# lh3/miniasm

Hardware: AMD Instinct MI355X
Metric: PAF overlaps processed/sec (hit-filter->trans-reduce->GFA) (higher is better)
Workload: dtype u32

## Files before the change

### include/mahip.h

```cpp
#ifndef MAHIP_H
#define MAHIP_H

#include <stddef.h>
#include <stdint.h>
#include "miniasm_amd.h"

#ifdef __cplusplus
extern "C" {
#endif

typedef struct mahip_ctx mahip_ctx_t;

int mahip_device_count(void);
mahip_ctx_t *mahip_create(int device, void *stream);
void mahip_destroy(mahip_ctx_t *c);
const char *mahip_strerror(void);
int mahip_sync(mahip_ctx_t *c);
int mahip_first_launch(mahip_ctx_t *c);

int mahip_hits_upload(mahip_ctx_t *c, const ma_hit_t *h, size_t n, uint32_t n_seq);
int mahip_hits_adopt(mahip_ctx_t *c, const void *d_hits, size_t n, uint32_t n_seq);
int mahip_set_shard(mahip_ctx_t *c, uint32_t q_beg, uint32_t q_end);
int mahip_hits_balance(mahip_ctx_t *c, int world, uint32_t *bounds);
int mahip_set_shard_bounds(mahip_ctx_t *c, const uint32_t *bounds, int world);
// ... 210 lines not shown
int mahip_useq_plan_last(mahip_ctx_t *c, mahip_useq_plan_info_t *info);
const char *mahip_useq_plan_reason_name(int reason);
int mahip_useq_plan_mem(mahip_ctx_t *c, uint32_t n_utg, const uint32_t *u_n, const uint32_t *u_len, const uint64_t *members, uint32_t n_seq, const char *blob, const uint64_t *off,
                        const void *sub, mahip_useq_plan_info_t *info);
int mahip_useq_plan_download(mahip_ctx_t *c, uint64_t *uoff, mahip_useq_place_t *pl, mahip_useq_want_t *want, char *names);
int mahip_useq_begin_planned(mahip_ctx_t *c);
int mahip_useq_place_text_planned(mahip_ctx_t *c, uint64_t *n_matched, uint64_t *n_dup, uint64_t *n_short, double *laps_ms);
int mahip_useq_stream_begin_planned(mahip_ctx_t *c);
enum { MAHIP_BGZF_OK = 0, MAHIP_BGZF_NOT_BGZF, MAHIP_BGZF_NO_BC, MAHIP_BGZF_PAST_END, MAHIP_BGZF_TRAILING, MAHIP_BGZF_BAD_FLG, MAHIP_BGZF_ISIZE,
       MAHIP_BGZF_BAD_BTYPE, MAHIP_BGZF_STORED_LEN, MAHIP_BGZF_BAD_LENGTHS, MAHIP_BGZF_BAD_SYMBOL, MAHIP_BGZF_DIST_TOO_FAR, MAHIP_BGZF_OUT_OVERFLOW, MAHIP_BGZF_IN_EXHAUSTED,
       MAHIP_BGZF_OUT_SHORT, MAHIP_BGZF_CRC, MAHIP_BGZF_NOMEM, MAHIP_BGZF_NOT_SEEKABLE, MAHIP_BGZF_FORCED, MAHIP_BGZF_EMPTY };
enum { MAHIP_BGZF_HOST = 1, MAHIP_BGZF_DEVICE = 2 };
enum { MAHIP_BGZF_PAF = 1, MAHIP_BGZF_FASTX = 2 };
typedef struct {
	uint64_t n_members, n_empty;
	uint64_t n_stored, n_fixed, n_dynamic;
	uint64_t comp_bytes, text_bytes;
	int reader, reason;
	int64_t first_bad_member;
	double laps_ms[4];
} mahip_bgzf_info_t;
typedef struct { uint64_t in_off, out_off; uint32_t in_len, isize, crc, pad; } mahip_bgzf_member_t;
int mahip_bgzf_load_fd(mahip_ctx_t *c, int fd, size_t nbytes, int target, mahip_bgzf_info_t *info);
int mahip_bgzf_load_mem(mahip_ctx_t *c, const void *comp, size_t nbytes, int target, mahip_bgzf_info_t *info);
int mahip_bgzf_inflate_mem(mahip_ctx_t *c, const void *comp, size_t ncomp, void *out, size_t out_cap, mahip_bgzf_info_t *info);
#define MAHIP_BGZF_RANGE_AHEAD 1
typedef struct {
	uint64_t text_bytes;
	uint64_t beg, end;
	uint64_t first_member, n_members_inflated;
	uint64_t comp_bytes_uploaded;
	int n_rounds;
} mahip_bgzf_range_t;
int mahip_bgzf_load_fd_range(mahip_ctx_t *c, int fd, size_t nbytes, int rank, int world, mahip_bgzf_range_t *range, mahip_bgzf_info_t *info);
int mahip_bgzf_range_mem(mahip_ctx_t *c, const void *comp, size_t ncomp, int rank, int world, void *out, size_t out_cap, mahip_bgzf_range_t *range, mahip_bgzf_info_t *info);
int mahip_text_first_nl(mahip_ctx_t *c, const void *d_text, uint64_t from, uint64_t to, uint64_t *pos);
int mahip_bgzf_last(mahip_ctx_t *c, mahip_bgzf_info_t *out);
void mahip_bgzf_note(mahip_ctx_t *c, const mahip_bgzf_info_t *in);
const char *mahip_bgzf_reason_name(int reason);
enum { MAHIP_GZIP_OK = 0, MAHIP_GZIP_BAD_HEADER, MAHIP_GZIP_MULTI_MEMBER, MAHIP_GZIP_NO_SYNC, MAHIP_GZIP_SYNC_MISMATCH, MAHIP_GZIP_ISIZE,
       MAHIP_GZIP_BAD_BTYPE, MAHIP_GZIP_STORED_LEN, MAHIP_GZIP_BAD_LENGTHS, MAHIP_GZIP_BAD_SYMBOL, MAHIP_GZIP_DIST_TOO_FAR, MAHIP_GZIP_OUT_OVERFLOW, MAHIP_GZIP_IN_EXHAUSTED,
       MAHIP_GZIP_OUT_SHORT, MAHIP_GZIP_CRC, MAHIP_GZIP_NOMEM, MAHIP_GZIP_NOT_SEEKABLE, MAHIP_GZIP_FORCED, MAHIP_GZIP_EMPTY };
#define MAHIP_GZIP_CHUNK_DEFAULT ((size_t)1 << 20)
typedef struct {
	uint64_t comp_bytes, text_bytes;
	uint64_t chunk, n_chunks, n_synced, n_items;
	uint64_t n_stored, n_fixed, n_dynamic;
	int reader, reason;
	int64_t first_bad_item;
	double laps_ms[6];
} mahip_gzip_info_t;
#define MAHIP_GZIP_SAW_FINAL 1u
#define MAHIP_GZIP_ON_CHAIN 2u
typedef struct {
	int64_t sync_bit;
	uint64_t end_bit, out_len;
	uint32_t status, flags;
} mahip_gzip_item_t;
int mahip_gzip_load_fd(mahip_ctx_t *c, int fd, size_t nbytes, int target, size_t chunk, mahip_gzip_info_t *info);
int mahip_gzip_load_mem(mahip_ctx_t *c, const void *comp, size_t nbytes, int target, size_t chunk, mahip_gzip_info_t *info);
int mahip_gzip_inflate_mem(mahip_ctx_t *c, const void *comp, size_t ncomp, size_t chunk, void *out, size_t out_cap, mahip_gzip_info_t *info);
int mahip_gzip_last(mahip_ctx_t *c, mahip_gzip_info_t *out);
void mahip_gzip_note(mahip_ctx_t *c, const mahip_gzip_info_t *in);
const char *mahip_gzip_reason_name(int reason);
uint64_t mahip_gzip_items_download(mahip_ctx_t *c, mahip_gzip_item_t *out, uint64_t cap);
uint32_t mahip_asg_n_arc(mahip_ctx_t *c);
enum { MAHIP_SCAN_ONE_TILE = 0, MAHIP_SCAN_CHAINED = 1, MAHIP_SCAN_THREE_PHASE = 2 };
void mahip_scan_forms(mahip_ctx_t *c, uint64_t out[3]);
int mahip_scan_u32(mahip_ctx_t *c, const uint32_t *d_in, uint32_t *d_out, size_t n, uint32_t *d_total);
uint64_t mahip_asg_trans_inner(mahip_ctx_t *c);
int mahip_asg_download(mahip_ctx_t *c, asg_t *g);

#define MAHIP_BUF_SUB0  0
#define MAHIP_BUF_SUB1  1
#define MAHIP_BUF_RCONT 2
#define MAHIP_BUF_RUSED 3
#define MAHIP_BUF_SDEL  4
int mahip_copy_out(mahip_ctx_t *c, int which, void *d_dst, size_t first, size_t count);
int mahip_copy_in(mahip_ctx_t *c, int which, const void *d_src, size_t first, size_t count);
int mahip_hits_contained_flags(mahip_ctx_t *c, const ma_opt_t *opt);
int mahip_hits_contained_finish(mahip_ctx_t *c, const uint8_t *seq_del, uint32_t *n_seq_new, size_t *n_live);
int mahip_sg_flags(mahip_ctx_t *c, const ma_opt_t *opt, int use_sub, const uint32_t *seq_len, const uint8_t *seq_del);
int mahip_sg_finish(mahip_ctx_t *c, uint32_t *n_arc);
int mahip_asg_export_rows(mahip_ctx_t *c, void *d_dst);
int mahip_asg_import_rows(mahip_ctx_t *c, const void *d_src, const uint32_t *counts, int n_ranks, size_t stride);
int mahip_set_full_input(mahip_ctx_t *c, int full);
int mahip_sg_push_conflicts(mahip_ctx_t *c, uint64_t *n_conf);
int mahip_sg_push_fix(mahip_ctx_t *c);
int mahip_asg_export_rows_push(mahip_ctx_t *c, void *d_dst);
int mahip_asg_import_push_rows(mahip_ctx_t *c, const void *d_src, const uint32_t *counts, int n_ranks, size_t stride);
int mahip_asg_del_trans_range(mahip_ctx_t *c, int fuzz, uint32_t v_beg, uint32_t v_end, uint32_t *n_reduced);
int mahip_asg_flags_out(mahip_ctx_t *c, void *d_dst, size_t first, size_t count);
int mahip_asg_flags_in(mahip_ctx_t *c, const void *d_src, size_t first, size_t count);
int mahip_asg_cleanup(mahip_ctx_t *c, uint32_t *n_arc);

int mahip_comm_unique_id(void *id128);
int mahip_comm_init(mahip_ctx_t *c, const void *id128, int rank, int world);
int mahip_comm_init_shm(mahip_ctx_t *c, const char *name, int rank, int world);
void mahip_comm_destroy(mahip_ctx_t *c);
int mahip_comm_rank(mahip_ctx_t *c);
int mahip_comm_world(mahip_ctx_t *c);
int mahip_comm_active(mahip_ctx_t *c);
int mahip_comm_all_gather(mahip_ctx_t *c, const void *d_send, void *d_recv, size_t bytes_per_rank);
int mahip_comm_all_reduce_max_u8(mahip_ctx_t *c, void *d_buf, size_t n);
int mahip_comm_all_reduce_sum_u64(mahip_ctx_t *c, uint64_t *h_vals, size_t n);
typedef struct {
	void *user;
	int (*all_gather)(void *user, const void *send, void *recv, size_t bytes);
	int (*all_reduce_max_u8)(void *user, void *buf, size_t n);
	int (*all_reduce_sum_u64)(void *user, uint64_t *vals, size_t n);
	int (*all_reduce_sum_u32)(void *user, void *buf, size_t n);
	int (*all_to_all_v)(void *user, const void *send, void *recv, const uint64_t *bytes);
} mahip_comm_ext_t;
int mahip_comm_init_ext(mahip_ctx_t *c, int rank, int world, const mahip_comm_ext_t *ext);
int mahip_comm_all_reduce_sum_u32(mahip_ctx_t *c, void *d_buf, size_t n);
int mahip_comm_all_to_all_v(mahip_ctx_t *c, const void *d_send, void *d_recv, const uint64_t *bytes);
int mahip_comm_all_gather_u64(mahip_ctx_t *c, const uint64_t *h_vals, size_t n, uint64_t *h_out);
int mahip_comm_barrier(mahip_ctx_t *c);
int mahip_xbuf(mahip_ctx_t *c, int slot, size_t bytes, void **d_ptr);

#define MAHIP_TEXT_PAF 1
#define MAHIP_TEXT_SG  2
#define MAHIP_TEXT_BED 3
#define MAHIP_TEXT_UG  4
#define MAHIP_TEXT_ROAD_HOST   1
#define MAHIP_TEXT_ROAD_DEVICE 2
#define MAHIP_TEXT_OK        0
#define MAHIP_TEXT_SWITCHED_OFF 1
#define MAHIP_TEXT_NOMEM     2
#define MAHIP_TEXT_NO_NAMES  3
#define MAHIP_TEXT_NO_UG     4
#define MAHIP_TEXT_NO_SEQ    5
#define MAHIP_TEXT_SEQ_NUL   6
#define MAHIP_TEXT_TOO_MANY  7
typedef struct {
	int kind, road, reason;
	uint64_t n_records;
	uint64_t n_lines;
	uint64_t text_bytes;
	uint64_t n_slabs, slab_records;
	uint64_t max_name;
	uint64_t n_slow_lines;
	double laps_ms[4];
	uint64_t n_seq_bytes;
	uint64_t seq_chunk;
} mahip_text_info_t;
typedef int (*mahip_text_sink_t)(void *arg, const char *text, size_t n);
int mahip_text_names(mahip_ctx_t *c, const char *blob, const uint64_t *off, uint32_t n_seq, const uint8_t *del);
int mahip_text_prepare(mahip_ctx_t *c, int kind, int have_sub, mahip_text_info_t *info);
int mahip_text_emit(mahip_ctx_t *c, mahip_text_sink_t sink, void *arg, mahip_text_info_t *info);
int mahip_text_dump(mahip_ctx_t *c, int kind, int have_sub, mahip_text_sink_t sink, void *arg, mahip_text_info_t *info);
int mahip_text_last(mahip_ctx_t *c, mahip_text_info_t *info);
int mahip_text_prepare_ug(mahip_ctx_t *c, int have_sub, const asg_arc_t *links, uint32_t n_links, int with_seq, mahip_text_info_t *info);
int mahip_text_format_mem(mahip_ctx_t *c, int kind, const void *records, uint64_t n_records, const void *sub, uint32_t n_seq, const uint8_t *del,
                          const char *blob, const uint64_t *off, uint64_t slab, char **text, size_t *len, mahip_text_info_t *info);
int mahip_text_format_ug_mem(mahip_ctx_t *c, uint32_t n_utg, const uint32_t *u_n, const uint32_t *u_len, const uint32_t *u_start, const uint32_t *u_end, const uint64_t *members,
                             const asg_arc_t *links, uint32_t n_links, const uint32_t *counts, const void *sub, uint32_t n_seq, int with_seq, const char *arena, uint64_t arena_bytes,
                             const char *blob, const uint64_t *off, uint64_t slab, char **text, size_t *len, mahip_text_info_t *info);
int mahip_text_enabled(void);

int mahip_prof_enable(mahip_ctx_t *c, int enable);
int mahip_prof_reset(mahip_ctx_t *c);
typedef struct { const char *name; uint64_t launches; double total_ms; double alg_bytes; } mahip_prof_t;
int mahip_prof_get(mahip_ctx_t *c, mahip_prof_t *out, int max);
int mahip_mark(mahip_ctx_t *c, int slot);
int mahip_marks_ms(mahip_ctx_t *c, int first, int n, float *ms);
// ... 17 lines not shown
```

### miniasm_amd/csrc/graph.hip

```cpp
#include "mahip_internal.hpp"
#include <type_traits>

#define DEAD 0x80000000u
#define ADEL 0x80000000u

struct HitColsG { const uint32_t *qid, *qs, *qe, *tn, *ts, *te, *ml, *bl; };
struct ArcCols { uint32_t *u, *v, *len, *ol; };

static HitColsG gcols_of(mahip_ctx *c)
{
	HitColsG h;
	h.qid = P<uint32_t>(c->col[0]); h.qs = P<uint32_t>(c->col[1]); h.qe = P<uint32_t>(c->col[2]); h.tn = P<uint32_t>(c->col[3]);
	h.ts = P<uint32_t>(c->col[4]); h.te = P<uint32_t>(c->col[5]); h.ml = P<uint32_t>(c->col[6]); h.bl = P<uint32_t>(c->col[7]);
	return h;
}
static ArcCols arcs_of(mahip_ctx *c, int g)
{
	ArcCols a;
	a.u = P<uint32_t>(c->au[g]); a.v = P<uint32_t>(c->av[g]); a.len = P<uint32_t>(c->alen[g]); a.ol = P<uint32_t>(c->aol[g]);
	return a;
}
static int reserve_arcs(mahip_ctx *c, size_t n)
{
	for (int g = 0; g < 2; ++g) {
		CHK(dev_reserve(c, c->au[g], (n + 4) * 4)); CHK(dev_reserve(c, c->av[g], (n + 4) * 4));
		CHK(dev_reserve(c, c->alen[g], (n + 4) * 4)); CHK(dev_reserve(c, c->aol[g], (n + 4) * 4));
	}
	CHK(dev_reserve(c, c->keep, (n + 16) * 4)); CHK(dev_reserve(c, c->pos, (n + 16) * 4));
	return 0;
}

__global__ __launch_bounds__(256) void k_sg_seq(const uint2 *__restrict__ sub, const uint8_t *__restrict__ r_del, const uint32_t *__restrict__ seq_len,
                                                 const uint8_t *__restrict__ seq_del, uint32_t n_seq, uint32_t *__restrict__ slen, uint8_t *__restrict__ sdel)
{
	uint32_t r = blockIdx.x * 256 + threadIdx.x;
	if (r >= n_seq) return;
	uint32_t len; int del;
	if (sub) { uint2 s = sub[r]; len = s.y - (s.x & 0x7fffffffu); del = s.x >> 31; }
	else len = seq_len[r], del = 0;
	if (seq_del) del |= seq_del[r];
	if (r_del) del |= r_del[r];
	slen[r] = len; sdel[r] = (uint8_t)del;
}

#define SG_TILE 16384u

__device__ __forceinline__ int sg_candidate(const HitColsG &h, size_t i, const uint32_t *__restrict__ slen, int max_hang, float int_frac, int min_ovlp,
                                            const uint8_t *__restrict__ lazy_del, mc_arc_t *x, uint32_t *q_, uint32_t *t_, int *self_rc)
{
	const uint32_t q = h.qid[i];
	if (lazy_del && lazy_del[q]) return -100;
	if (h.bl[i] & DEAD) return -100;
	const uint32_t t = h.tn[i];
	if (lazy_del && lazy_del[t]) return -100;
	uint32_t qs = h.qs[i], qe = h.qe[i], ts = h.ts[i], te = h.te[i];
	int rev = h.ml[i] >> 31;
	*q_ = q; *t_ = t;
	*self_rc = q == t && qs == ts && qe == te && rev;
	return mc_hit2arc(q, qs, qe, t, ts, te, rev, (int)slen[q], (int)slen[t], max_hang, int_frac, min_ovlp, x);
}

__global__ __launch_bounds__(256) void k_sg_arcs(HitColsG h, size_t n, const uint32_t *__restrict__ slen, uint8_t *__restrict__ sdel,
                                                  int max_hang, float int_frac, int min_ovlp, unsigned long long *__restrict__ ctr, const uint8_t *__restrict__ lazy_del,
                                                  unsigned long long *__restrict__ cmask)
{
	uint32_t mx = 0, n_live = 0;
	for (size_t base = (size_t)blockIdx.x * 256; base < n; base += (size_t)gridDim.x * 256) {
		const size_t i = base + threadIdx.x;
		int cand = 0;
		if (i < n) {
			mc_arc_t x;
			uint32_t q = 0, t = 0;
			int self_rc = 0, r = sg_candidate(h, i, slen, max_hang, int_frac, min_ovlp, lazy_del, &x, &q, &t, &self_rc);
			if (r != -100) {
				++n_live;
				if (r >= 0) {
					if (q == t) { if (self_rc) sdel[q] = 1; }
					else cand = 1, mx = x.len > mx ? x.len : mx;
				} else if (r == MC_HT_QCONT) sdel[q] = 1;
			}
		}
		const unsigned long long m = wv_ballot(cand);
		if ((threadIdx.x & 63) == 0) cmask[i >> 6] = m;
	}
	blk_max_u64(&ctr[CT_MAXLEN], mx);
	blk_add_u64(&ctr[CT_LIVE], n_live);
}

#ifndef SG_DENSE
#define SG_DENSE 6
#endif
__device__ __forceinline__ unsigned long long wv_bcast_u64(unsigned long long x, int src) { return (unsigned long long)__shfl((uint32_t)(x >> 32), src, 64) << 32 | __shfl((uint32_t)x, src, 64); }

__global__ __launch_bounds__(256) void k_sg_emit(HitColsG h, size_t n, const uint32_t *__restrict__ slen, const uint8_t *__restrict__ sdel,
                                                  int max_hang, float int_frac, int min_ovlp, const unsigned long long *cmask,
                                                  uint32_t *__restrict__ tile_cnt, const uint32_t *__restrict__ tile_off, ArcCols out, uint32_t *__restrict__ aslot,
                                                  uint32_t *__restrict__ wpos, unsigned long long *kmask)
{
	__shared__ uint32_t s_w[4];
	const unsigned lane = threadIdx.x & 63;
	const size_t w = (size_t)blockIdx.x * 256 + threadIdx.x, n_words = (n + 63) >> 6, w0 = w - lane;
	unsigned long long m = w < n_words ? cmask[w] : 0ull, kept = 0;
	uint32_t cnt = 0;
	const bool dense = __popcll(m) >= SG_DENSE;
	const unsigned long long dense_lanes = wv_ballot(dense);
	for (unsigned long long dl = dense_lanes; dl; dl &= dl - 1) {
		const int l = __ffsll((long long)dl) - 1;
		const unsigned long long ml = wv_bcast_u64(m, l);
		const size_t i = ((w0 + (size_t)l) << 6) + lane;
		const int k = (ml >> lane & 1ull) && i < n && !sdel[h.qid[i]] && !sdel[h.tn[i]];
		const unsigned long long kb = wv_ballot(k);
		if ((int)lane == l) kept = kb, cnt = (uint32_t)__popcll(kb);
	}
	if (!dense)
		for (unsigned long long rest = m; rest; rest &= rest - 1) {
			const int b = __ffsll((long long)rest) - 1;
			const size_t i = (w << 6) + (size_t)b;
			if (i < n && !sdel[h.qid[i]] && !sdel[h.tn[i]]) kept |= 1ull << b, ++cnt;
		}
	uint32_t tot, ex = block_excl_scan_256(cnt, s_w, &tot);
	if (!out.u) { if (threadIdx.x == 0) tile_cnt[blockIdx.x] = tot; return; }
	uint32_t p = tile_off[blockIdx.x] + ex;
	if (wpos && w < n_words) { wpos[w] = p; kmask[w] = kept; }
	for (unsigned long long dl = dense_lanes; dl; dl &= dl - 1) {
		const int l = __ffsll((long long)dl) - 1;
		const unsigned long long kl = wv_bcast_u64(kept, l);
		const uint32_t pl = __shfl(p, l, 64);
		if (kl >> lane & 1ull) {
			const size_t i = ((w0 + (size_t)l) << 6) + lane;
			const uint32_t pp = pl + (uint32_t)__popcll(kl & wv_lt(lane));
			mc_arc_t x;
			uint32_t q = 0, t = 0;
			int self_rc = 0;
			sg_candidate(h, i, slen, max_hang, int_frac, min_ovlp, nullptr, &x, &q, &t, &self_rc);
			out.u[pp] = x.u; out.v[pp] = x.v; out.len[pp] = x.len; out.ol[pp] = x.ol;
			if (aslot) aslot[pp] = (uint32_t)i;
		}
	}
	if (!dense)
		for (; kept; kept &= kept - 1, ++p) {
			const size_t i = (w << 6) + (size_t)(__ffsll((long long)kept) - 1);
			mc_arc_t x;
			uint32_t q = 0, t = 0;
			int self_rc = 0;
			sg_candidate(h, i, slen, max_hang, int_frac, min_ovlp, nullptr, &x, &q, &t, &self_rc);
			out.u[p] = x.u; out.v[p] = x.v; out.len[p] = x.len; out.ol[p] = x.ol;
			if (aslot) aslot[p] = (uint32_t)i;
		}
}

__global__ __launch_bounds__(256) void k_arc_keep(ArcCols a, size_t n, const uint8_t *__restrict__ sdel, uint32_t *__restrict__ keep, int use_keep_in)
{
	size_t i = (size_t)blockIdx.x * 256 + threadIdx.x;
	if (i >= n) return;
	int k = use_keep_in ? (int)keep[i] : 1;
	if (k) k = !(a.ol[i] & ADEL) && !sdel[a.u[i] >> 1] && !sdel[a.v[i] >> 1];
	keep[i] = k;
}

__global__ __launch_bounds__(256) void k_arc_compact(ArcCols in, size_t n, const uint32_t *__restrict__ keep, const uint32_t *__restrict__ pos, ArcCols out)
{
	size_t i = (size_t)blockIdx.x * 256 + threadIdx.x;
	if (i < n && keep[i]) {
		uint32_t p = pos[i];
		out.u[p] = in.u[i]; out.v[p] = in.v[i]; out.len[p] = in.len[i]; out.ol[p] = in.ol[i];
	}
}
// ... 697 lines not shown
}
__global__ __launch_bounds__(256) void k_arc_rows_in(const uint4 *__restrict__ rows, size_t n, size_t dst0, ArcCols a)
{
	size_t i = (size_t)blockIdx.x * 256 + threadIdx.x;
	if (i < n) { uint4 r = rows[i]; a.u[dst0 + i] = r.x; a.v[dst0 + i] = r.y; a.len[dst0 + i] = r.z; a.ol[dst0 + i] = r.w; }
}

__global__ __launch_bounds__(256) void k_rows_permute(const uint4 *__restrict__ in, size_t n, const uint32_t *__restrict__ perm, uint4 *__restrict__ out)
{
	size_t i = (size_t)blockIdx.x * 256 + threadIdx.x;
	if (i < n) out[i] = in[perm[i]];
}

uint32_t graph_nseq(const mahip_ctx *c) { return c->gsq ? c->n_seq_new : c->n_seq; }
static const int32_t *graph_map(mahip_ctx *c) { return c->has_map && !c->gsq ? (const int32_t*)P<int32_t>(c->map) : (const int32_t*)nullptr; }

static int arc_reindex(mahip_ctx *c)
{
	size_t V = 2 * (size_t)graph_nseq(c);
	CHK(dev_reserve(c, c->idx, (V + 2) * 8));
	HIPCHK(hipMemsetAsync(c->idx.p, 0, V * 8, c->st));
	if (c->n_arc) {
		ProfScope ps(c, "k_arc_index", 16.0 * (double)c->n_arc);
		hipLaunchKernelGGL(k_arc_index, dim3(grid_for(c->n_arc, 256)), dim3(256), 0, c->st, (const uint32_t*)P<uint32_t>(c->au[c->ag]), (size_t)c->n_arc, P<unsigned long long>(c->idx));
	}
	HIPCHK(hipGetLastError());
	return 0;
}

static int arc_cleanup(mahip_ctx *c, size_t n_in, int keep_in, int index_mode)
{
	uint32_t *d_tot = (uint32_t*)(P<unsigned long long>(c->ctr) + CT_TOTAL);
	if (n_in == 0) { c->n_arc = 0; return index_mode < 0 ? 0 : arc_reindex(c); }
	ArcCols in = arcs_of(c, c->ag), out = arcs_of(c, c->ag ^ 1);
	if (!keep_in) {
		ProfScope ps(c, "k_arc_rm", 32.0 * (double)n_in);
		if (c->arcs_clean) {
			const size_t ng = (n_in + RMC_GROUP - 1) / RMC_GROUP;
			hipLaunchKernelGGL(k_arc_rm_count, dim3((unsigned)ng), dim3(256), 0, c->st, (const uint32_t*)in.ol, n_in, P<uint32_t>(c->keep));
			CHK(scan_exclusive_u32(c, P<uint32_t>(c->keep), P<uint32_t>(c->pos), ng, d_tot));
			hipLaunchKernelGGL(k_arc_rm_write, dim3((unsigned)ng), dim3(256), 0, c->st, in, n_in, out, (const uint32_t*)P<uint32_t>(c->pos));
		} else {
			const size_t nb = (n_in + RM_TILE - 1) / RM_TILE;
			uint32_t *ticket; unsigned long long *state; uint32_t ticket_base, epoch;
			CHK(scan_chain_begin(c, nb, &state, &ticket, &ticket_base, &epoch));
			hipLaunchKernelGGL(k_arc_rm_chain, dim3((unsigned)nb), dim3(256), 0, c->st, in, n_in, (const uint8_t*)P<uint8_t>(c->sdel), out, d_tot, state, ticket, ticket_base, epoch);
		}
	} else {
		ProfScope ps(c, "k_arc_rm", 32.0 * (double)n_in);
		hipLaunchKernelGGL(k_arc_keep, dim3(grid_for(n_in, 256)), dim3(256), 0, c->st, in, n_in, (const uint8_t*)P<uint8_t>(c->sdel), P<uint32_t>(c->keep), keep_in);
		CHK(scan_exclusive_u32(c, P<uint32_t>(c->keep), P<uint32_t>(c->pos), n_in, d_tot));
		hipLaunchKernelGGL(k_arc_compact, dim3(grid_for(n_in, 256)), dim3(256), 0, c->st, in, n_in, (const uint32_t*)P<uint32_t>(c->keep), (const uint32_t*)P<uint32_t>(c->pos), out);
	}
	CHK(ctr_fetch(c));
	uint32_t n_out = (uint32_t)(c->h_ctr[CT_TOTAL] & 0xffffffffu);
	c->ag ^= 1;
	int changed = n_out != n_in;
	c->n_arc = n_out;
	c->arcs_clean = true;
	if (index_mode > 0 || (index_mode == 0 && changed)) CHK(arc_reindex(c));
	return 0;
}


extern "C" int mahip_sg_flags(mahip_ctx_t *c, const ma_opt_t *opt, int use_sub, const uint32_t *seq_len, const uint8_t *seq_del)
{
	HIPCHK(hipSetDevice(c->dev));
	CHK(hits_need_cols(c, "mahip_sg_gen"));
	size_t n = c->n_hits;
	uint32_t R = c->n_seq;
	CHK(dev_reserve(c, c->slen, ((size_t)R + 4) * 4)); CHK(dev_reserve(c, c->sdel, (size_t)R + 16));
	c->sg_max_hang = opt->max_hang; c->sg_int_frac = opt->int_frac; c->sg_min_ovlp = opt->min_ovlp;
	c->gsq = false; c->arcs_clean = false;
	CHK(ctr_zero(c));
	unsigned long long *ctr = P<unsigned long long>(c->ctr);
	const uint32_t *d_len = nullptr; const uint8_t *d_del = nullptr;
	if (seq_len) { CHK(dev_reserve(c, c->big0, ((size_t)R + 4) * 4)); HIPCHK(hipMemcpyAsync(c->big0.p, seq_len, (size_t)R * 4, hipMemcpyHostToDevice, c->st)); d_len = P<uint32_t>(c->big0); }
	if (seq_del) { CHK(dev_reserve(c, c->big1, (size_t)R + 16)); HIPCHK(hipMemcpyAsync(c->big1.p, seq_del, R, hipMemcpyHostToDevice, c->st)); d_del = P<uint8_t>(c->big1); }
	if (!use_sub && !d_len) { mahip_set_error("mahip_sg_gen: need sub or seq_len"); return -1; }
	if (R) hipLaunchKernelGGL(k_sg_seq, dim3(grid_for(R, 256)), dim3(256), 0, c->st, use_sub ? (const uint2*)P<uint2>(c->sub[0]) : (const uint2*)nullptr,
	                          c->has_map ? (const uint8_t*)P<uint8_t>(c->r_del) : (const uint8_t*)nullptr, d_len, d_del, R, P<uint32_t>(c->slen), P<uint8_t>(c->sdel));
	c->ag = 0;
	if (n) CHK(dev_reserve(c, c->sgmask, (n / 64 + 8) * 8));
	if (n) {
		ProfScope ps(c, "k_sg_arcs", 64.0 * (double)c->n_live);
		hipLaunchKernelGGL(k_sg_arcs, dim3(grid_for(n, 256, MA_STREAM_BLOCKS)), dim3(256), 0, c->st, gcols_of(c), n, (const uint32_t*)P<uint32_t>(c->slen), P<uint8_t>(c->sdel),
		                   opt->max_hang, opt->int_frac, opt->min_ovlp, ctr,
		                   c->lazy_squeeze ? (const uint8_t*)P<uint8_t>(c->r_del) : (const uint8_t*)nullptr, P<unsigned long long>(c->sgmask));
	}
	HIPCHK(hipGetLastError());
	return 0;
}

static int push_stable_order(mahip_ctx *c, size_t m, int *gen, uint64_t *conflicts)
{
	unsigned long long *ctr = P<unsigned long long>(c->ctr);
	const int bs = hits_qs_bits(c);
	int bq = 0;
	for (uint64_t x = c->n_seq ? c->n_seq - 1 : 0xffffffffull; x; x >>= 1) ++bq;
	for (int k = 0; k < 2; ++k) { CHK(dev_reserve(c, c->key[k], (m + 1) * 8)); CHK(dev_reserve(c, c->val[k], (m + 1) * 4)); }
	hipLaunchKernelGGL(k_arc_slot_keys, dim3(grid_for(m, 256)), dim3(256), 0, c->st, (const uint32_t*)P<uint32_t>(c->aslot), m, c->d_aos, (const uint32_t*)P<uint32_t>(c->sidx),
	                   P<uint64_t>(c->key[0]), P<uint32_t>(c->val[0]));
	*gen = 0;
	CHK(radix_sort_pairs(c, m, 0, bs, 32, 32 + (bq ? bq : 1), gen));
	HIPCHK(hipMemsetAsync(ctr + ST_PUSH_CONFLICTS, 0, 8, c->st));
	hipLaunchKernelGGL(k_arc_push_conflicts, dim3(grid_for(m, 256, MA_STREAM_BLOCKS)), dim3(256), 0, c->st, (const uint64_t*)P<uint64_t>(c->key[*gen]), m, ctr);
	CHK(ctr_fetch(c));
	*conflicts = c->h_ctr[ST_PUSH_CONFLICTS];
	return 0;
}

static int push_order(mahip_ctx *c, size_t m, bool exact, int *gen, const ArcCols *pushed = nullptr, const ArcCols *sorted = nullptr)
{
	uint64_t conf = 0;
	bool want_known = false;
	TieLaps tl(c);
	CHK(push_stable_order(c, m, gen, &conf));
	tl.lap("stable push order + conflicts");
	c->tie.push_conflicts = conf;
	c->tie.push_conflicts_seen = conf;
	static const bool filter_on = !(getenv("MA_TIE_NO_FILTER") && atoi(getenv("MA_TIE_NO_FILTER")) != 0);
	if (exact && conf && pushed && sorted && filter_on && m < 0xffffffffull) {
		unsigned long long *ctr = P<unsigned long long>(c->ctr);
		const int32_t *map = c->has_map ? (const int32_t*)P<int32_t>(c->map) : (const int32_t*)nullptr;
		uint64_t *S = P<uint64_t>(c->key[*gen ^ 1]);
		CHK(dev_reserve(c, c->keep, (m + 16) * 4)); CHK(dev_reserve(c, c->pos, (m + 16) * 4));
		hipLaunchKernelGGL(k_arc_keys_ref, dim3(grid_for(m, 256)), dim3(256), 0, c->st, *sorted, m, map, S);
		hipLaunchKernelGGL(k_tie_pair_flags, dim3(grid_for(m, 256)), dim3(256), 0, c->st, (const uint64_t*)S, m, P<uint32_t>(c->keep));
		CHK(scan_exclusive_u32(c, P<uint32_t>(c->keep), P<uint32_t>(c->pos), m, nullptr));
		HIPCHK(hipMemsetAsync(ctr + ST_PUSH_SEEN, 0, 8, c->st));
		const size_t want_bytes = ((size_t)c->n_seq / 32 + 2) * 4;
		CHK(dev_reserve(c, c->wantb, want_bytes));
		HIPCHK(hipMemsetAsync(c->wantb.p, 0, want_bytes, c->st));
		hipLaunchKernelGGL(k_arc_push_conflicts_seen, dim3(grid_for(m, 256, MA_STREAM_BLOCKS)), dim3(256), 0, c->st, (const uint64_t*)P<uint64_t>(c->key[*gen]), (const uint32_t*)P<uint32_t>(c->val[*gen]),
		                   *pushed, map, (const uint64_t*)S, (const uint32_t*)P<uint32_t>(c->pos), (uint32_t)m, ctr, P<uint32_t>(c->wantb));
		CHK(ctr_fetch(c));
		c->tie.push_conflicts_seen = c->h_ctr[ST_PUSH_SEEN];
		want_known = true;
		tl.lap("conflicts the arc sort can see");
	}
	if (exact && c->tie.push_conflicts_seen) {
		const int g_keep = *gen; (void)g_keep;
		static const bool walk_all = getenv("MA_TIE_WALK_ALL") && atoi(getenv("MA_TIE_WALK_ALL")) != 0;
		CHK(hits_reference_rank(c, false, want_known && !walk_all));
		for (int k = 0; k < 2; ++k) { CHK(dev_reserve(c, c->key[k], (m + 1) * 8)); CHK(dev_reserve(c, c->val[k], (m + 1) * 4)); }
		hipLaunchKernelGGL(k_arc_push_keys, dim3(grid_for(m, 256)), dim3(256), 0, c->st, (const uint32_t*)P<uint32_t>(c->aslot), (const uint32_t*)P<uint32_t>(c->hrank), m,
		                   P<uint64_t>(c->key[0]), P<uint32_t>(c->val[0]));
		*gen = 0;
		int bh = 0;
		for (uint64_t x = c->n_in; x; x >>= 1) ++bh;
		CHK(radix_sort_pairs(c, m, 0, bh ? bh : 1, 0, 0, gen));
	}
	return 0;
}

extern "C" int mahip_sg_finish(mahip_ctx_t *c, uint32_t *n_arc)
{
	HIPCHK(hipSetDevice(c->dev));
	size_t n = c->n_hits;
	uint32_t R = c->n_seq;
	CHK(ctr_fetch(c));
	c->n_live = (size_t)c->h_ctr[CT_LIVE];
	if (c->prof) prof_patch_last(c, "k_sg_arcs", 64.0 * (double)c->n_live);
	c->n_arc = 0; c->ag = 0;
	const bool sharded = c->q_beg > 0 || (c->n_seq && c->q_end < c->n_seq);
	const bool want_slots = c->sorted_here && c->sidx.p != nullptr;
	const int blen = bitlen_u64(c->h_ctr[CT_MAXLEN]);
	{ const uint64_t keep_hit_ties = c->tie.hit_ties; const int keep_walk = c->hrank_ready; memset(&c->tie, 0, sizeof(c->tie)); c->tie.hit_ties = keep_hit_ties; c->tie.hit_walk = keep_walk; }
	if (n) {
		const size_t n_tiles = (n + SG_TILE - 1) / SG_TILE;
		const unsigned long long *lazy = (const unsigned long long*)P<unsigned long long>(c->sgmask);
		uint32_t *d_tot = (uint32_t*)(P<unsigned long long>(c->ctr) + CT_TOTAL);
		ArcCols none = { nullptr, nullptr, nullptr, nullptr };
		CHK(dev_reserve(c, c->keep, (n + 16) * 4)); CHK(dev_reserve(c, c->pos, (n + 16) * 4));
		{
			ProfScope ps(c, "k_sg_emit", 4.0 * (double)n + 64.0 * (double)c->n_live);
			hipLaunchKernelGGL(k_sg_emit, dim3((unsigned)n_tiles), dim3(256), 0, c->st, gcols_of(c), n, (const uint32_t*)P<uint32_t>(c->slen), (const uint8_t*)P<uint8_t>(c->sdel),
			                   c->sg_max_hang, c->sg_int_frac, c->sg_min_ovlp, lazy, P<uint32_t>(c->keep), (const uint32_t*)nullptr, none, (uint32_t*)nullptr, (uint32_t*)nullptr, (unsigned long long*)nullptr);
		}
		CHK(scan_exclusive_u32(c, P<uint32_t>(c->keep), P<uint32_t>(c->pos), n_tiles, d_tot));
		CHK(ctr_fetch(c));
		c->n_arc = (uint32_t)(c->h_ctr[CT_TOTAL] & 0xffffffffu);
		CHK(reserve_arcs(c, c->n_arc));
		if (want_slots) CHK(dev_reserve(c, c->aslot, ((size_t)c->n_arc + 4) * 4));
		CHK(dev_reserve(c, c->apos, (n / 64 + 8) * 4));
		if (c->n_arc) {
			ProfScope ps(c, "k_sg_emit", 4.0 * (double)n + 64.0 * (double)c->n_live + 16.0 * (double)c->n_arc);
			hipLaunchKernelGGL(k_sg_emit, dim3((unsigned)n_tiles), dim3(256), 0, c->st, gcols_of(c), n, (const uint32_t*)P<uint32_t>(c->slen), (const uint8_t*)P<uint8_t>(c->sdel),
			                   c->sg_max_hang, c->sg_int_frac, c->sg_min_ovlp, lazy, (uint32_t*)nullptr, (const uint32_t*)P<uint32_t>(c->pos), arcs_of(c, 0),
			                   want_slots ? P<uint32_t>(c->aslot) : (uint32_t*)nullptr, P<uint32_t>(c->apos), P<unsigned long long>(c->sgmask));
		}
	} else CHK(reserve_arcs(c, 0));
	c->n_push = 0; c->push_ordered = false;
	if (sharded && c->tie_mode != 0) {
		CHK(dev_reserve(c, c->pushrows[0], ((size_t)c->n_arc + 1) * 16));
		if (c->n_arc) hipLaunchKernelGGL(k_arc_rows_out, dim3(grid_for(c->n_arc, 256)), dim3(256), 0, c->st, arcs_of(c, c->ag), (size_t)c->n_arc, (uint4*)c->pushrows[0].p);
		c->n_push = c->n_arc;
	}
	if (c->n_arc > 1) {
		size_t m = c->n_arc;
		for (int k = 0; k < 2; ++k) { CHK(dev_reserve(c, c->key[k], (m + 1) * 8)); CHK(dev_reserve(c, c->val[k], (m + 1) * 4)); }
		ArcCols in = arcs_of(c, c->ag), out = arcs_of(c, c->ag ^ 1);
		unsigned long long *ctr = P<unsigned long long>(c->ctr);
		const int32_t *map = c->has_map ? (const int32_t*)P<int32_t>(c->map) : (const int32_t*)nullptr;
		int gen = 0, need_walk = c->tie_mode == 1 && !sharded;
		TieLaps tl(c);
		if (c->tie_mode == 0 && want_slots) {
			int g0 = 0;
			CHK(push_order(c, m, false, &g0));
			hipLaunchKernelGGL(k_arc_permute, dim3(grid_for(m, 256)), dim3(256), 0, c->st, in, m, (const uint32_t*)P<uint32_t>(c->val[g0]), out);
			c->ag ^= 1;
			in = arcs_of(c, c->ag); out = arcs_of(c, c->ag ^ 1);
		}
		bool idx_done = false;
		if (c->tie_mode != 1 || sharded) {
			bool fast = blen + AG_IB + 1 <= 31 && !getenv("MA_ARC_RADIX");
			if (fast) {
				const size_t V = 2 * (size_t)R;
				const uint32_t q_lo = sharded ? c->q_beg : 0u, q_hi = sharded && c->q_end < R ? c->q_end : R, Rr = q_hi > q_lo ? q_hi - q_lo : 1;
				CHK(dev_reserve(c, c->idx, (V + 2) * 8));
				HIPCHK(hipMemsetAsync(c->idx.p, 0, V * 8, c->st));
				HIPCHK(hipMemsetAsync(ctr + CT_OVF2, 0, 8, c->st));
				HIPCHK(hipMemsetAsync(ctr + CT_STICKY, 0, (64 - CT_STICKY) * 8, c->st));
				{
					ProfScope ps(c, "k_arc_group_sort", 48.0 * (double)m);
					const unsigned grid = grid_for(((size_t)Rr + 63) / 64, 4, MA_STREAM_BLOCKS);
					const uint32_t *goff = (const uint32_t*)P<uint32_t>(c->goff), *wpos = (const uint32_t*)P<uint32_t>(c->apos);
					const unsigned long long *km = (const unsigned long long*)P<unsigned long long>(c->sgmask);
					hipLaunchKernelGGL(k_arc_group_sort<true>, dim3(grid), dim3(256), 0, c->st, in, out, goff, wpos, km, (uint32_t)n, (uint32_t)m, q_lo, q_hi, blen ? blen : 1, P<unsigned long long>(c->idx), ctr);
					hipLaunchKernelGGL(k_arc_group_sort<false>, dim3(grid), dim3(256), 0, c->st, in, out, goff, wpos, km, (uint32_t)n, (uint32_t)m, q_lo, q_hi, blen ? blen : 1, P<unsigned long long>(c->idx), ctr);
				}
				CHK(ctr_fetch(c));
				if (c->h_ctr[CT_OVF2]) fast = false;
				else {
					idx_done = true;
					if (c->tie_mode == 2 && !sharded) {
						c->tie.arc_tie_groups = c->h_ctr[ST_ARC_TIE_GROUPS]; c->tie.arc_tie_arcs = c->h_ctr[ST_ARC_TIE_ARCS];
						need_walk = c->tie.arc_tie_groups > 0;
					}
				}
			}
			if (!fast) {
			hipLaunchKernelGGL(k_arc_keys, dim3(grid_for(m, 256)), dim3(256), 0, c->st, in, m, P<uint64_t>(c->key[0]), P<uint32_t>(c->val[0]));
			c->radix_arcs = true;
			CHK(radix_sort_pairs(c, m, 0, blen, 32, 32 + bitlen_u64(2ull * R), &gen));
			c->radix_arcs = false;
			{
				ProfScope ps(c, "k_arc_permute", 36.0 * (double)m);
				hipLaunchKernelGGL(k_arc_permute, dim3(grid_for(m, 256)), dim3(256), 0, c->st, in, m, (const uint32_t*)P<uint32_t>(c->val[gen]), out);
			}
			if (c->tie_mode == 2 && !sharded) {
				HIPCHK(hipMemsetAsync(ctr + CT_STICKY, 0, (64 - CT_STICKY) * 8, c->st));
				ProfScope ps(c, "k_arc_tie_census", 8.0 * (double)m);
				hipLaunchKernelGGL(k_arc_tie_census, dim3(grid_for(m, 256, MA_STREAM_BLOCKS)), dim3(256), 0, c->st, (const uint64_t*)P<uint64_t>(c->key[gen]), m, ctr);
				CHK(ctr_fetch(c));
				c->tie.arc_tie_groups = c->h_ctr[ST_ARC_TIE_GROUPS]; c->tie.arc_tie_arcs = c->h_ctr[ST_ARC_TIE_ARCS];
				need_walk = c->tie.arc_tie_groups > 0;
			}
			}
			tl.lap("stable arc sort + census");
		}
		if (need_walk) {
			if (want_slots) {
				int g2 = 0;
				const bool have_sorted = c->tie_mode != 1 || sharded;
				CHK(push_order(c, m, true, &g2, &in, have_sorted ? &out : nullptr));
				hipLaunchKernelGGL(k_arc_permute, dim3(grid_for(m, 256)), dim3(256), 0, c->st, in, m, (const uint32_t*)P<uint32_t>(c->val[g2]), out);
				c->ag ^= 1;
				in = arcs_of(c, c->ag); out = arcs_of(c, c->ag ^ 1);
				tl.lap("push order (all of it)");
			}
			hipLaunchKernelGGL(k_arc_keys_ref, dim3(grid_for(m, 256)), dim3(256), 0, c->st, in, m, map, P<uint64_t>(c->key[0]));
			CHK(reference_order(c, P<uint64_t>(c->key[0]), m, P<uint32_t>(c->val[1])));
			{
				ProfScope ps(c, "k_arc_permute", 36.0 * (double)m);
				hipLaunchKernelGGL(k_arc_permute, dim3(grid_for(m, 256)), dim3(256), 0, c->st, in, m, (const uint32_t*)P<uint32_t>(c->val[1]), out);
			}
			c->tie.arc_walk = 1;
			tl.lap("arc walk (all of it)");
			walk_scratch_release(c);
			idx_done = false;
		}
		c->ag ^= 1;
		if (!idx_done) CHK(arc_reindex(c));
	} else CHK(arc_reindex(c));
	HIPCHK(hipGetLastError());
	c->graph_ready = true;
	c->arcs_clean = true;
	if (n_arc) *n_arc = c->n_arc;
	return 0;
}

extern "C" int mahip_sg_gen(mahip_ctx_t *c, const ma_opt_t *opt, int use_sub, const uint32_t *seq_len, const uint8_t *seq_del, uint32_t *n_arc)
{
	CHK(mahip_sg_flags(c, opt, use_sub, seq_len, seq_del));
	return mahip_sg_finish(c, n_arc);
}

extern "C" int mahip_asg_export_rows(mahip_ctx_t *c, void *d_dst)
{
	HIPCHK(hipSetDevice(c->dev));
	if (!c->graph_ready) { mahip_set_error("mahip_asg_export_rows: no graph"); return -1; }
	if (c->n_arc) hipLaunchKernelGGL(k_arc_rows_out, dim3(grid_for(c->n_arc, 256)), dim3(256), 0, c->st, arcs_of(c, c->ag), (size_t)c->n_arc, (uint4*)d_dst);
	if (xchg_needs_sync(c)) HIPCHK(hipStreamSynchronize(c->st));
	return 0;
}

extern "C" int mahip_asg_import_rows(mahip_ctx_t *c, const void *d_src, const uint32_t *counts, int n_ranks, size_t stride)
{
	HIPCHK(hipSetDevice(c->dev));
	size_t tot = 0;
	for (int r = 0; r < n_ranks; ++r) tot += counts[r];
	if (tot >= 0x7fffffffull) { mahip_set_error("mahip_asg_import_rows: too many arcs"); return -1; }
	CHK(reserve_arcs(c, tot));
	c->ag = 0; c->gsq = false; c->arcs_clean = false;
	ArcCols a = arcs_of(c, 0);
	size_t off = 0;
	for (int r = 0; r < n_ranks; ++r) {
		if (counts[r]) hipLaunchKernelGGL(k_arc_rows_in, dim3(grid_for(counts[r], 256)), dim3(256), 0, c->st, (const uint4*)d_src + (size_t)r * stride, (size_t)counts[r], off, a);
		off += counts[r];
	}
	c->n_arc = (uint32_t)tot;
	CHK(arc_reindex(c));
	memset(&c->tie, 0, sizeof(c->tie));
	if (c->tie_mode != 0 && tot > 1) {
		unsigned long long *ctr = P<unsigned long long>(c->ctr);
		CHK(dev_reserve(c, c->key[0], (tot + 1) * 8)); CHK(dev_reserve(c, c->val[0], (tot + 1) * 4));
		hipLaunchKernelGGL(k_arc_keys, dim3(grid_for(tot, 256)), dim3(256), 0, c->st, a, tot, P<uint64_t>(c->key[0]), P<uint32_t>(c->val[0]));
		HIPCHK(hipMemsetAsync(ctr + CT_STICKY, 0, (64 - CT_STICKY) * 8, c->st));
		hipLaunchKernelGGL(k_arc_tie_census, dim3(grid_for(tot, 256, MA_STREAM_BLOCKS)), dim3(256), 0, c->st, (const uint64_t*)P<uint64_t>(c->key[0]), tot, ctr);
		CHK(ctr_fetch(c));
		c->tie.arc_tie_groups = c->h_ctr[ST_ARC_TIE_GROUPS]; c->tie.arc_tie_arcs = c->h_ctr[ST_ARC_TIE_ARCS];
		c->tie.unrepaired = c->tie.arc_tie_groups > 0;
	}
	if (xchg_needs_sync(c)) HIPCHK(hipStreamSynchronize(c->st));
	c->graph_ready = true;
	return 0;
}

extern "C" int mahip_sg_push_conflicts(mahip_ctx_t *c, uint64_t *n_conf)
{
	HIPCHK(hipSetDevice(c->dev));
	*n_conf = 0;
	const size_t m = c->n_push;
	CHK(dev_reserve(c, c->pushrows[1], (m + 1) * 16));
	if (m < 2 || !c->aslot.p || !c->sidx.p) {
		if (m) HIPCHK(hipMemcpyAsync(c->pushrows[1].p, c->pushrows[0].p, m * 16, hipMemcpyDeviceToDevice, c->st));
		c->push_ordered = true;
		return 0;
	}
	int g = 0;
	CHK(push_stable_order(c, m, &g, n_conf));
	hipLaunchKernelGGL(k_rows_permute, dim3(grid_for(m, 256)), dim3(256), 0, c->st, (const uint4*)c->pushrows[0].p, m, (const uint32_t*)P<uint32_t>(c->val[g]), (uint4*)c->pushrows[1].p);
	HIPCHK(hipGetLastError());
	c->push_ordered = true;
	return 0;
}

extern "C" int mahip_sg_push_fix(mahip_ctx_t *c)
{
	HIPCHK(hipSetDevice(c->dev));
	const size_t m = c->n_push;
	if (m < 2) return 0;
	CHK(hits_reference_rank(c, true));
	for (int k = 0; k < 2; ++k) { CHK(dev_reserve(c, c->key[k], (m + 1) * 8)); CHK(dev_reserve(c, c->val[k], (m + 1) * 4)); }
	CHK(dev_reserve(c, c->pushrows[1], (m + 1) * 16));
	hipLaunchKernelGGL(k_arc_push_keys, dim3(grid_for(m, 256)), dim3(256), 0, c->st, (const uint32_t*)P<uint32_t>(c->aslot), (const uint32_t*)P<uint32_t>(c->hrank), m, P<uint64_t>(c->key[0]), P<uint32_t>(c->val[0]));
	int g = 0;
	CHK(radix_sort_pairs(c, m, 0, 32, 0, 0, &g));
	hipLaunchKernelGGL(k_rows_permute, dim3(grid_for(m, 256)), dim3(256), 0, c->st, (const uint4*)c->pushrows[0].p, m, (const uint32_t*)P<uint32_t>(c->val[g]), (uint4*)c->pushrows[1].p);
	HIPCHK(hipGetLastError());
	c->push_ordered = true;
	return 0;
}

// ... 323 lines not shown
```

### miniasm_amd/csrc/mahip_internal.hpp

```cpp
#pragma once
#include <hip/hip_runtime.h>
#include <stdint.h>
#include <stdio.h>
#include <stdlib.h>
#include <string.h>
#include <time.h>
#include <vector>
#include <mutex>
#include <string>
#include "mahip.h"
#include "ma_core.h"

void mahip_set_error(const char *fmt, ...);
extern "C" int ma_timing_level(void);

#define HIPCHK(expr) do { hipError_t e_ = (expr); if (e_ != hipSuccess) { \
	mahip_set_error("%s:%d: %s -> %s", __FILE__, __LINE__, #expr, hipGetErrorString(e_)); return -1; } } while (0)
#define CHK(expr) do { int r_ = (expr); if (r_ != 0) return r_; } while (0)

struct DevBuf {
	void *p = nullptr;
	size_t cap = 0;
	bool ext = false;
};

struct ProfEvent { const char *name; hipEvent_t a, b; double alg_bytes; };
struct ProfAcc { const char *name; uint64_t launches; double ms; double alg_bytes; };

struct DevPool {
	struct Base { char *p; size_t bytes; };
	struct Piece { char *p; size_t cap; char *base; };
	std::vector<Base> bases;
	std::vector<Piece> free_pieces;
	std::mutex mu;
};

struct BigHost { void *p = nullptr; size_t bytes = 0; bool mapped = false; bool reserve(size_t n); void drop(); };

struct mahip_ctx {
	int dev = 0;
	hipStream_t st = nullptr;
	bool own_stream = false;
	size_t mem_bytes = 0;
	DevPool pool;

	size_t n_hits = 0;
	size_t n_in = 0;
	bool full_input = true;
	DevBuf gpos;
	uint64_t n_total = 0;
	size_t n_live = 0;
	uint32_t n_seq = 0;
	uint32_t q_beg = 0, q_end = 0xffffffffu;
	std::vector<uint32_t> shard_bounds;
	uint32_t hint_max_qs = 0;
	uint32_t paf_max_qs = 0;
	const ma_hit_t *d_aos = nullptr;
	DevBuf aos_own;
	DevBuf col[8];
	DevBuf goff;
	DevBuf sub[2];
	DevBuf r_cont, r_used, r_del, r_live;
	DevBuf map;
	DevBuf surv;
	bool soa_ready = false, has_map = false, lazy_squeeze = false;
	bool surv_ready = false;
	int sg_max_hang = 0, sg_min_ovlp = 0; float sg_int_frac = 0;
	int tie_mode = 2;
	DevBuf sidx;
	DevBuf hrank;
	DevBuf orank;
	DevBuf aslot;
	DevBuf apos;
	DevBuf pushrows[2];
	uint32_t n_push = 0;
	bool sorted_here = false, hrank_ready = false, orank_ready = false;
	bool gather_pending = false; int gk_gen = 0, gk_bi = 0;
	bool gk_runs = false; size_t n_runs = 0; int run_stride = 0;
	bool push_ordered = false;
	mahip_tie_info_t tie = {0, 0, 0, 0, 0, 0, 0, 0, 0};
	uint32_t n_seq_new = 0;

	DevBuf au[2], av[2], alen[2], aol[2];
	int ag = 0;
	uint32_t n_arc = 0;
	DevBuf idx;
	DevBuf sdel;
	DevBuf slen;
	bool graph_ready = false;
	bool gsq = false;
	void *comm = nullptr;
	DevBuf xb[2];
	void *clean = nullptr;
	void *ug = nullptr;
	void *useq = nullptr;
	void *text = nullptr;

	DevBuf keep, pos;
	BigHost hwalk, hdig;
	DevBuf tdig;
	DevBuf wantb;
	DevBuf wseg;
	DevBuf key[2], val[2];
	DevBuf hist;
	DevBuf scan_tmp[3];
	DevBuf gs_tmp;
	DevBuf ctr;
	DevBuf ovf;
	DevBuf big0, big1;
	DevBuf marks;
	DevBuf sgmask;
	uint64_t *h_ctr = nullptr;
	unsigned long long ctr_seq = 0;
	uint32_t scan_ticket = 0, scan_epoch = 0;
	void *xfer = nullptr;
	mahip_xfer_info_t xfer_last = {};
	void *paf = nullptr;
	bool paf_keep_odd = false;
	mahip_bgzf_info_t bgzf_last = {};
	mahip_gzip_info_t gzip_last = {};
	mahip_gzip_item_t *gzip_rows = nullptr;
	uint64_t gzip_n_rows = 0;

	hipEvent_t mark_ev[64] = {};
	hipStream_t sub_side[2] = {}; hipEvent_t sub_ev[3] = {};
	uint64_t scan_forms[3] = {0, 0, 0};
	mahip_sort_info_t sort_last = {};
	struct { int n_pass, bits[16], shift[16]; uint32_t fixed7; int groups; } rs_last = {};
	uint64_t tr_inner = 0;
	bool arcs_clean = false;
	bool radix_arcs = false;
	bool sub_fork_failed = false;
	unsigned long long mark_set = 0;
	bool prof = false;
	std::vector<ProfEvent> pev;
	std::vector<size_t> pstack;
	std::vector<ProfAcc> pacc;
};

int dev_reserve(mahip_ctx *c, DevBuf &b, size_t bytes);
void dev_free(mahip_ctx *c, DevBuf &b);
void prof_begin(mahip_ctx *c, const char *name, double alg_bytes);
void prof_end(mahip_ctx *c);
int prof_collect(mahip_ctx *c);
void prof_patch_last(mahip_ctx *c, const char *name, double alg_bytes);

struct ProfScope {
	mahip_ctx *c;
	ProfScope(mahip_ctx *c_, const char *name, double alg_bytes) : c(c_) { if (c->prof) prof_begin(c, name, alg_bytes); }
	~ProfScope() { if (c->prof) prof_end(c); }
};

struct TieLaps {
	mahip_ctx *c; bool on; double t0 = 0;
	static double now() { struct timespec ts; clock_gettime(CLOCK_MONOTONIC, &ts); return ts.tv_sec + ts.tv_nsec * 1e-9; }
	explicit TieLaps(mahip_ctx *c_) : c(c_) { on = ma_timing_level() >= 2; if (on) { (void)hipStreamSynchronize(c->st); t0 = now(); } }
	void lap(const char *what) { if (!on) return; (void)hipStreamSynchronize(c->st); const double t1 = now(); fprintf(stderr, "[T::ties]   %-34s %9.3f ms\n", what, (t1 - t0) * 1e3); t0 = t1; }
};
// ... 289 lines not shown
```

Baseline: 6.291 billion.

## Sweep only surviving reads' hit segments when generating string-graph arc candidates

Adds a survivor-driven sweep for the arc candidate pass. When lazy squeezing leaves few surviving reads relative to the total, each wave walks the contiguous hit ranges of a batch of surviving queries via goff, and sets candidate bits with atomics in a pre-zeroed mask. Previously the kernel scanned every hit. Per-block partial max and live counts are folded by a second kernel. It also adds host download helpers for flags and slots. The cost is a memset, atomics and irregular gathers in exchange for skipping dead hits.

```diff
diff --git a/include/mahip.h b/include/mahip.h
--- a/include/mahip.h
+++ b/include/mahip.h
@@ -316,6 +316,8 @@
 int mahip_hits_contained_finish(mahip_ctx_t *c, const uint8_t *seq_del, uint32_t *n_seq_new, size_t *n_live);
 int mahip_sg_flags(mahip_ctx_t *c, const ma_opt_t *opt, int use_sub, const uint32_t *seq_len, const uint8_t *seq_del);
 int mahip_sg_finish(mahip_ctx_t *c, uint32_t *n_arc);
+int mahip_sg_flags_download(mahip_ctx_t *c, uint64_t *cmask, uint8_t *sdel, uint64_t *max_len, uint64_t *n_live, int *surv_sweep);
+int mahip_sg_slots_download(mahip_ctx_t *c, uint32_t *aslot);
 int mahip_asg_export_rows(mahip_ctx_t *c, void *d_dst);
 int mahip_asg_import_rows(mahip_ctx_t *c, const void *d_src, const uint32_t *counts, int n_ranks, size_t stride);
 int mahip_set_full_input(mahip_ctx_t *c, int full);
diff --git a/miniasm_amd/csrc/graph.hip b/miniasm_amd/csrc/graph.hip
--- a/miniasm_amd/csrc/graph.hip
+++ b/miniasm_amd/csrc/graph.hip
@@ -44,6 +44,7 @@
 }
 
 #define SG_TILE 16384u
+#define SG_SURV_FRAC 4u
 
 __device__ __forceinline__ int sg_candidate(const HitColsG &h, size_t i, const uint32_t *__restrict__ slen, int max_hang, float int_frac, int min_ovlp,
                                             const uint8_t *__restrict__ lazy_del, mc_arc_t *x, uint32_t *q_, uint32_t *t_, int *self_rc)
@@ -83,6 +84,84 @@
 		const unsigned long long m = wv_ballot(cand);
 		if ((threadIdx.x & 63) == 0) cmask[i >> 6] = m;
 	}
+	blk_max_u64(&ctr[CT_MAXLEN], mx);
+	blk_add_u64(&ctr[CT_LIVE], n_live);
+}
+
+#ifndef SGS_BATCH
+#define SGS_BATCH 8
+#endif
+#ifndef SGS_UNROLL
+#define SGS_UNROLL 4
+#endif
+__global__ __launch_bounds__(256) void k_sg_arcs_surv(HitColsG h, const uint32_t *__restrict__ goff, const uint32_t *__restrict__ surv, uint32_t n_surv,
+                                                       const uint32_t *__restrict__ slen, uint8_t *__restrict__ sdel, int max_hang, float int_frac, int min_ovlp,
+                                                       unsigned long long *__restrict__ part , const uint8_t *__restrict__ lazy_del,
+                                                       unsigned long long *__restrict__ cmask)
+{
+	const unsigned lane = threadIdx.x & 63;
+	const uint32_t stride = gridDim.x * 4 * SGS_BATCH;
+	uint32_t mx = 0, n_live = 0;
+	for (uint32_t k0 = (blockIdx.x * 4 + (threadIdx.x >> 6)) * SGS_BATCH; k0 < n_surv; k0 += stride) {
+		const bool has = lane < SGS_BATCH && k0 + lane < n_surv;
+		const uint32_t q_l = has ? surv[k0 + lane] : 0u;
+		uint32_t beg_l = 0, cnt_l = 0, lq_l = 0;
+		if (has) { beg_l = goff[q_l]; cnt_l = goff[q_l + 1] - beg_l; lq_l = slen[q_l]; }
+		uint32_t inc = cnt_l;
+#pragma unroll
+		for (int d = 1; d < SGS_BATCH; d <<= 1) { const uint32_t y = __shfl_up(inc, d, 64); if ((int)lane >= d) inc += y; }
+		const uint32_t ex_l = inc - cnt_l, total = __shfl(inc, SGS_BATCH - 1, 64);
+		uint32_t ex[SGS_BATCH];
+#pragma unroll
+		for (int k = 0; k < SGS_BATCH; ++k) ex[k] = (uint32_t)__builtin_amdgcn_readlane((int)ex_l, k);
+		for (uint32_t j0 = 0; j0 < total; j0 += 64 * SGS_UNROLL) {
+			bool in[SGS_UNROLL];
+			uint32_t i[SGS_UNROLL];
+			uint32_t q[SGS_UNROLL], lq[SGS_UNROLL], bl[SGS_UNROLL], t[SGS_UNROLL], qs[SGS_UNROLL], qe[SGS_UNROLL], ts[SGS_UNROLL], te[SGS_UNROLL], ml[SGS_UNROLL], lt[SGS_UNROLL];
+			uint8_t t_gone[SGS_UNROLL];
+#pragma unroll
+			for (int u = 0; u < SGS_UNROLL; ++u) {
+				const uint32_t j = j0 + (uint32_t)u * 64 + lane;
+				in[u] = j < total;
+				int s = 0;
+#pragma unroll
+				for (int k = 1; k < SGS_BATCH; ++k) s += j >= ex[k];
+				q[u] = __shfl(q_l, s, 64); lq[u] = __shfl(lq_l, s, 64);
+				const uint32_t beg_s = __shfl(beg_l, s, 64), ex_s = __shfl(ex_l, s, 64);
+				i[u] = in[u] ? beg_s + (j - ex_s) : 0u;
+				bl[u] = in[u] ? h.bl[i[u]] : DEAD;
+				t[u] = h.tn[i[u]]; qs[u] = h.qs[i[u]]; qe[u] = h.qe[i[u]]; ts[u] = h.ts[i[u]]; te[u] = h.te[i[u]]; ml[u] = h.ml[i[u]];
+			}
+#pragma unroll
+			for (int u = 0; u < SGS_UNROLL; ++u) { const uint32_t tt = bl[u] & DEAD ? q[u] : t[u]; t_gone[u] = lazy_del[tt]; lt[u] = slen[tt]; }
+#pragma unroll
+			for (int u = 0; u < SGS_UNROLL; ++u) {
+				if ((bl[u] & DEAD) || t_gone[u]) continue;
+				mc_arc_t x;
+				const int rev = ml[u] >> 31;
+				const int r = mc_hit2arc(q[u], qs[u], qe[u], t[u], ts[u], te[u], rev, (int)lq[u], (int)lt[u], max_hang, int_frac, min_ovlp, &x);
+				++n_live;
+				if (r >= 0) {
+					if (q[u] == t[u]) { if (qs[u] == ts[u] && qe[u] == te[u] && rev) sdel[q[u]] = 1; }
+					else { atomicOr(&cmask[i[u] >> 6], 1ull << (i[u] & 63)); mx = x.len > mx ? x.len : mx; }
+				} else if (r == MC_HT_QCONT) sdel[q[u]] = 1;
+			}
+		}
+	}
+	__shared__ unsigned long long s_mx[4], s_live[4];
+	const unsigned long long wmx = wv_max_u64(mx), wlive = wv_sum_u64(n_live);
+	if (lane == 0) { s_mx[threadIdx.x >> 6] = wmx; s_live[threadIdx.x >> 6] = wlive; }
+	__syncthreads();
+	if (threadIdx.x == 0) {
+		unsigned long long m = 0, l = 0;
+		for (int w = 0; w < 4; ++w) { m = s_mx[w] > m ? s_mx[w] : m; l += s_live[w]; }
+		part[2 * (size_t)blockIdx.x] = m; part[2 * (size_t)blockIdx.x + 1] = l;
+	}
+}
+__global__ __launch_bounds__(256) void k_sg_arcs_fold(const unsigned long long *__restrict__ part, uint32_t n_blocks, unsigned long long *__restrict__ ctr)
+{
+	unsigned long long mx = 0, n_live = 0;
+	for (uint32_t b = threadIdx.x; b < n_blocks; b += 256) { const unsigned long long m = part[2 * (size_t)b]; mx = m > mx ? m : mx; n_live += part[2 * (size_t)b + 1]; }
 	blk_max_u64(&ctr[CT_MAXLEN], mx);
 	blk_add_u64(&ctr[CT_LIVE], n_live);
 }
@@ -946,7 +1025,21 @@
 	                          c->has_map ? (const uint8_t*)P<uint8_t>(c->r_del) : (const uint8_t*)nullptr, d_len, d_del, R, P<uint32_t>(c->slen), P<uint8_t>(c->sdel));
 	c->ag = 0;
 	if (n) CHK(dev_reserve(c, c->sgmask, (n / 64 + 8) * 8));
-	if (n) {
+	CHK(dev_reserve(c, c->keep, (size_t)MA_STREAM_BLOCKS * 16 + 64));
+	const bool sharded = c->q_beg > 0 || (c->n_seq && c->q_end < c->n_seq);
+	const bool surv_sweep = n && c->lazy_squeeze && c->has_map && c->sorted_here && !sharded && !seq_len && !seq_del && (uint64_t)c->n_seq_new * SG_SURV_FRAC <= R;
+	c->sg_surv_sweep = surv_sweep;
+	if (surv_sweep) {
+		ProfScope ps(c, "k_sg_arcs", 64.0 * (double)c->n_live);
+		HIPCHK(hipMemsetAsync(c->sgmask.p, 0, ((n + 63) / 64) * 8, c->st));
+		if (c->n_seq_new) {
+			const unsigned nb = grid_for(c->n_seq_new, 4 * SGS_BATCH, MA_STREAM_BLOCKS);
+			hipLaunchKernelGGL(k_sg_arcs_surv, dim3(nb), dim3(256), 0, c->st, gcols_of(c), (const uint32_t*)P<uint32_t>(c->goff),
+			                   (const uint32_t*)P<uint32_t>(c->surv), c->n_seq_new, (const uint32_t*)P<uint32_t>(c->slen), P<uint8_t>(c->sdel),
+			                   opt->max_hang, opt->int_frac, opt->min_ovlp, P<unsigned long long>(c->keep), (const uint8_t*)P<uint8_t>(c->r_del), P<unsigned long long>(c->sgmask));
+			hipLaunchKernelGGL(k_sg_arcs_fold, dim3(1), dim3(256), 0, c->st, (const unsigned long long*)P<unsigned long long>(c->keep), nb, ctr);
+		}
+	} else if (n) {
 		ProfScope ps(c, "k_sg_arcs", 64.0 * (double)c->n_live);
 		hipLaunchKernelGGL(k_sg_arcs, dim3(grid_for(n, 256, MA_STREAM_BLOCKS)), dim3(256), 0, c->st, gcols_of(c), n, (const uint32_t*)P<uint32_t>(c->slen), P<uint8_t>(c->sdel),
 		                   opt->max_hang, opt->int_frac, opt->min_ovlp, ctr,
@@ -1056,6 +1149,7 @@
 		}
 	} else CHK(reserve_arcs(c, 0));
 	c->n_push = 0; c->push_ordered = false;
+	c->n_aslot = want_slots ? c->n_arc : 0;
 	if (sharded && c->tie_mode != 0) {
 		CHK(dev_reserve(c, c->pushrows[0], ((size_t)c->n_arc + 1) * 16));
 		if (c->n_arc) hipLaunchKernelGGL(k_arc_rows_out, dim3(grid_for(c->n_arc, 256)), dim3(256), 0, c->st, arcs_of(c, c->ag), (size_t)c->n_arc, (uint4*)c->pushrows[0].p);
@@ -1155,6 +1249,28 @@
 	return 0;
 }
 
+extern "C" int mahip_sg_flags_download(mahip_ctx_t *c, uint64_t *cmask, uint8_t *sdel, uint64_t *max_len, uint64_t *n_live, int *surv_sweep)
+{
+	HIPCHK(hipSetDevice(c->dev));
+	CHK(ctr_fetch(c));
+	if (cmask && c->n_hits) HIPCHK(hipMemcpyAsync(cmask, c->sgmask.p, ((c->n_hits + 63) / 64) * 8, hipMemcpyDeviceToHost, c->st));
+	if (sdel && c->n_seq) HIPCHK(hipMemcpyAsync(sdel, c->sdel.p, c->n_seq, hipMemcpyDeviceToHost, c->st));
+	HIPCHK(hipStreamSynchronize(c->st));
+	if (max_len) *max_len = c->h_ctr[CT_MAXLEN];
+	if (n_live) *n_live = c->h_ctr[CT_LIVE];
+	if (surv_sweep) *surv_sweep = c->sg_surv_sweep;
+	return 0;
+}
+
+extern "C" int mahip_sg_slots_download(mahip_ctx_t *c, uint32_t *aslot)
+{
+	HIPCHK(hipSetDevice(c->dev));
+	if (!c->graph_ready) { mahip_set_error("mahip_sg_slots_download: no graph"); return -1; }
+	if (c->n_aslot) HIPCHK(hipMemcpyAsync(aslot, c->aslot.p, (size_t)c->n_aslot * 4, hipMemcpyDeviceToHost, c->st));
+	HIPCHK(hipStreamSynchronize(c->st));
+	return 0;
+}
+
 extern "C" int mahip_sg_gen(mahip_ctx_t *c, const ma_opt_t *opt, int use_sub, const uint32_t *seq_len, const uint8_t *seq_del, uint32_t *n_arc)
 {
 	CHK(mahip_sg_flags(c, opt, use_sub, seq_len, seq_del));
diff --git a/miniasm_amd/csrc/mahip_internal.hpp b/miniasm_amd/csrc/mahip_internal.hpp
--- a/miniasm_amd/csrc/mahip_internal.hpp
+++ b/miniasm_amd/csrc/mahip_internal.hpp
@@ -66,6 +66,7 @@
 	bool soa_ready = false, has_map = false, lazy_squeeze = false;
 	bool surv_ready = false;
 	int sg_max_hang = 0, sg_min_ovlp = 0; float sg_int_frac = 0;
+	bool sg_surv_sweep = false;
 	int tie_mode = 2;
 	DevBuf sidx;
 	DevBuf hrank;
@@ -74,6 +75,7 @@
 	DevBuf apos;
 	DevBuf pushrows[2];
 	uint32_t n_push = 0;
+	uint32_t n_aslot = 0;
 	bool sorted_here = false, hrank_ready = false, orank_ready = false;
 	bool gather_pending = false; int gk_gen = 0, gk_bi = 0;
 	bool gk_runs = false; size_t n_runs = 0; int run_stride = 0;
```

After: 6.458 billion, median of 6. +2.7%, better.
